# KudanLimited/cuda-bundle-adjustment

Hardware: AMD Instinct MI355X
Metric: ba_edge_iterations_per_sec (higher is better)
Workload: dtype f64

## Files before the change

cuda-bundle-adjustment_amd/csrc/host/engine.cpp:

```cpp
#include "engine.h"

#include <algorithm>
#include <atomic>
#include <chrono>
#include <cmath>
#include <cstring>
#include <cstdio>
#include <cstdlib>
#include <memory>
#include <thread>

#include "../kernels/kernels.h"
#include "chol_solver.h"
#include "edge_layout.h"
#include "hip_util.h"
#include "options.h"
#include "rccl_comm.h"
#include "relpose_plan.h"
#include "schur_plan.h"
#include "structure_gpu.h"
#include "thread_pool.h"

namespace cugo_host
{
// ... 1301 lines not shown
        m.pe.bind_relpose_plan(m.hsc_rowptr, m.hsc_colind, s, false);
    }
    m.begin_call(true);
    const Impl::CallFacts& f = m.f;
    Impl::LmState& st = m.st = Impl::LmState{};
    auto sync_prof = [&](int item, Clock::time_point t0) {
        if (m.profile)
        {
            CUGO_HIP(hipStreamSynchronize(s));
            prof_[item] += ms_since(t0);
        }
    };
    m.hash_begin(niterations);

    for (int iteration = 0; iteration < niterations; iteration++)
    {
        const auto it0 = Clock::now();
        auto tb = Clock::now();
        if (!st.spec_queued)
            m.queue_build(m.cur, f.can_fuse && iteration > 0 ? lambda : -1.0, iteration == 0 ? m.d_scal.data() : nullptr);
        st.spec_queued = false;
        sync_prof(PROF_BUILD_SYSTEM, tb);
        if (iteration == 0)
        {
            const double* hpp = m.d_Hpp.data();
            if (f.sharded)
            {
                CUGO_HIP(hipMemcpyAsync(m.d_tmp.data(), m.d_Hpp.data(), 36 * (size_t)m.P * sizeof(double),
                                        hipMemcpyDeviceToDevice, s));
                m.exchange(m.d_tmp.data(), 36 * (size_t)m.P, 0);
                hpp = m.d_tmp.data();
            }
            cugo_k::launch_max_diagonal(s, hpp, m.P, m.d_Hll.data(), m.L, m.rs(), m.d_scal.data() + 1);
            if (f.sharded)
            {
                m.exchange(m.d_scal.data(), 1, 0);
                m.exchange(m.d_scal.data() + 1, 1, 1);
            }
            CUGO_HIP(hipMemcpyAsync(m.h_scal.data(), m.d_scal.data(), 2 * sizeof(double), hipMemcpyDeviceToHost, s));
            CUGO_HIP(hipStreamSynchronize(s));
            F = m.h_scal[0];
            lambda = tau * m.h_scal[1];
        }

        int q = 0;
        double rho = -1.0;
        for (; q < maxq && rho < 0; q++)
        {
            const int hash_it = q == 0 ? iteration : -1;
            const bool trial_fused = q == 0 && st.fused_lambda == lambda;
            const bool one_stream = trial_fused && f.ps_on;
            if (st.spec_queued || (!one_stream && !st.hpp_valid))
            {
                m.queue_build(m.cur, -1.0);
                st.spec_queued = false;
            }
            m.hash(hash_it, 0, m.d_Hpp.data(), 36 * (size_t)m.P);
            m.hash(hash_it, 1, m.d_b.data(), 6 * (size_t)m.P + 3 * (size_t)m.L);
            m.hash(hash_it, 2, m.d_Hll.data(), 9 * (size_t)m.L);
            m.hash(hash_it, 3, m.d_Hpl.data(), f.blkw);
            auto ts = Clock::now();
            if (!(trial_fused && st.schur_lambda == lambda))
                m.queue_schur(lambda, trial_fused, one_stream, m.cur);
            st.schur_lambda = -1.0;
            if (f.sharded)
                m.exchange_system();
            sync_prof(PROF_SCHUR, ts);
            m.hash(hash_it, 4, m.d_sys.data(), 36 * (size_t)m.hs.n_blocks + 6 * (size_t)m.P);
            if (m.d_T.size())
                m.hash(hash_it, 5, m.d_T.data(), f.blkw);
            m.hash(hash_it, 6, m.d_invHll.data(), 9 * (size_t)m.L);
            auto tn = Clock::now();
            m.queue_factor_solve(lambda, hash_it);
            sync_prof(PROF_NUMERIC, tn);
            m.hash(hash_it, 7, m.xp(), 6 * (size_t)m.P);
            auto tu = Clock::now();
            const int nxt = m.cur ^ 1;
            int n_scale_part = 0;
            m.timed("backsubst_update", [&] {
                n_scale_part = cugo_k::launch_backsubst_update(
                    s, m.ev, lambda, (m.rank == 0 ? lambda : 0.0), m.d_invHll.data(), m.bl(), m.bp(),
                    one_stream ? m.d_T.data() : m.d_Hpl.data(), m.xp(), m.xl(), m.d_poses[m.cur].data(), m.d_lms[m.cur].data(),
                    m.d_poses[nxt].data(), m.d_lms[nxt].data(), m.rs(), f.sharded ? m.d_scal.data() + 3 : nullptr,
                    one_stream ? m.d_lmrec.data() : nullptr);
            });
            sync_prof(PROF_UPDATE, tu);
            m.hash(hash_it, 8, m.xl(), 3 * (size_t)m.L);
            m.hash(hash_it, 9, m.d_poses[nxt].data(), 7 * (size_t)m.Pall);
            m.hash(hash_it, 10, m.d_lms[nxt].data(), 3 * (size_t)m.Lall);
            auto te = Clock::now();
            const double lambda_pred = lambda * (1.0 / 3.0);
            const double fuse_pred = f.can_fuse ? lambda_pred : -1.0;
            const bool last = iteration + 1 == niterations;
            const bool from_build = f.from_build && q == 0 && !last && st.prev_clamped;
            if (from_build)
            {
                m.queue_build(nxt, fuse_pred, nullptr, true);
                m.timed("errors", [&] {
                    int n_icp_chi = 0;
                    const double* icp_chi = m.pe.chi_totals(&n_icp_chi);
                    cugo_k::launch_trial_tail_from_build(s, m.ev, m.rs(), n_scale_part, m.d_scal.data() + 2,
                                                         m.d_scal.data() + 4, m.h_scal.data() + 2, (double)++m.trial_seq,
                                                         reinterpret_cast<unsigned*>(m.d_fail.data() + 2), icp_chi,
                                                         n_icp_chi);
                });
                if (f.can_fuse)
                {
                    m.queue_schur(lambda_pred, true, f.ps_on, nxt);
                    st.schur_lambda = lambda_pred;
                }
                st.spec_queued = true;
            }
            else
            m.timed("errors", [&] {
                if (f.sharded)
                    cugo_k::launch_errors(s, m.ev, m.d_poses[nxt].data(), m.d_lms[nxt].data(), m.rk,
                                          m.rs(), m.d_scal.data() + 2);
                else
                {
                    int n_icp_chi = 0;
                    const double* icp_chi = m.pe.chi_totals(&n_icp_chi);
                    m.pe.queue_errors(s, m.d_poses[nxt].data());
                    cugo_k::launch_errors_tail(s, m.ev, m.d_poses[nxt].data(), m.d_lms[nxt].data(), m.rk, m.rs(),
                                               n_scale_part, m.d_scal.data() + 2, m.d_scal.data() + 4,
                                               m.h_scal.data() + 2, (double)++m.trial_seq,
                                               reinterpret_cast<unsigned*>(m.d_fail.data() + 2), icp_chi, n_icp_chi);
                }
            });
            m.last_err_buf = nxt;
            sync_prof(PROF_COMPUTE_ERROR, te);
            if (!from_build && f.speculate && q == 0 && !last)
            {
                if (!f.trial_poll && f.trial_event)
                {
                    if (!m.trial_ev)
                        CUGO_HIP(hipEventCreateWithFlags(&m.trial_ev, hipEventDisableTiming));
                    CUGO_HIP(hipEventRecord(m.trial_ev, s));
                }
                m.queue_build(nxt, fuse_pred);
                st.spec_queued = true;
            }
            const bool flag_summed = f.sharded && m.chol.own_subtrees();
            if (f.sharded)
            {
                if (flag_summed)
                    cugo_k::launch_flag_to_double(s, m.d_fail_flag());
                m.exchange(m.d_scal.data() + 2, flag_summed ? 3 : 2, 0);
                CUGO_HIP(hipMemcpyAsync(m.h_scal.data() + 2, m.d_scal.data() + 2, 3 * sizeof(double),
                                        hipMemcpyDeviceToHost, s));
            }
            m.wait_for_trial(st.spec_queued, sstats_.trial_sync_retries);
            int32_t fail_flag;
            std::memcpy(&fail_flag, m.h_scal.data() + 4, sizeof fail_flag);
            if (flag_summed)
                fail_flag = m.h_scal[4] > 0.5 ? 1 : 0;
            const bool success = fail_flag == 0;
            const double Fhat = m.h_scal[2];
            const double scale = (success ? m.h_scal[3] : 0.0) + 1e-3;
            const double Fdiff = Fhat - F;
            rho = success ? (F - Fhat) / scale : -1.0;
            if (!success)
                std::printf("factorize failed!\n");
            if (rho > 0)
            {
                const double a = 1 - std::pow(2 * rho - 1, 3);
                lambda *= std::max(1.0 / 3.0, std::min(a, 2.0 / 3.0));
                st.prev_clamped = a <= 1.0 / 3.0;
// ... 201 lines not shown
```

cuda-bundle-adjustment_amd/csrc/host/options.h:

```cpp
#pragma once
#include <cstdlib>

namespace cugo_host
{

struct Options
{
    int hsc_mfma = 1;
    bool hsc_xcd = true;
    bool hsc_rows = false, hsc_strip = false, schur_plan = false;
    bool fuse_t = true;
    bool pose_schur = true;
    bool float32 = false;
    bool speculate = true, trial_event = true, trial_poll = true;
    bool trial_from_build = true;
    bool profile = false;
    bool init_timing = false;
    bool structure_reuse = true;
    bool flatten_reuse = true;
    bool async_structure = true;
    bool host_structure = false;
    bool upload_thread = true;
    int own_subtrees = -1;
    double own_min_gflop = 3.0;
    bool lookahead = false;
    bool ea_lds = true, panel16 = true, asm_fronts = true;
    bool ea_direct = true;
    bool bw_chain = true;
    bool reduce_scatter = true;

    static Options from_env()
    {
        Options o;
        auto flag = [](const char* name) { return std::getenv(name) != nullptr; };
        auto off = [](const char* name) {
            const char* e = std::getenv(name);
            return e && e[0] == '0';
        };
        auto on = [](const char* name) {
            const char* e = std::getenv(name);
            return e && e[0] == '1';
        };
        if (const char* e = std::getenv("CUGO_HSC_MFMA"))
            o.hsc_mfma = e[0] == '0' ? 0 : e[0] == '2' ? 2 : 1;
        o.hsc_xcd = !off("CUGO_HSC_XCD");
        o.schur_plan = flag("CUGO_SCHUR_PLAN");
        o.hsc_rows = on("CUGO_HSC_ROWS"), o.hsc_strip = on("CUGO_HSC_STRIP");
        o.fuse_t = !off("CUGO_FUSE_T");
        o.pose_schur = !off("CUGO_POSE_SCHUR");
        o.float32 = on("CUGO_FLOAT32");
        o.speculate = !off("CUGO_SPECULATE"), o.trial_event = !off("CUGO_TRIAL_EVENT"), o.trial_poll = !off("CUGO_TRIAL_POLL");
        o.trial_from_build = !off("CUGO_TRIAL_FROM_BUILD");
        o.profile = flag("CUGO_PROFILE");
        o.init_timing = flag("CUGO_INIT_TIMING");
        o.structure_reuse = !flag("CUGO_NO_STRUCTURE_REUSE");
        o.flatten_reuse = !flag("CUGO_NO_FLATTEN_REUSE");
        o.async_structure = !off("CUGO_ASYNC_STRUCTURE");
        o.host_structure = flag("CUGO_HOST_STRUCTURE");
        o.upload_thread = !off("CUGO_UPLOAD_THREAD");
        if (const char* e = std::getenv("CUGO_OWN_SUBTREES"))
            o.own_subtrees = e[0] == '1' ? 1 : e[0] == '0' ? 0 : -1;
        if (const char* e = std::getenv("CUGO_OWN_MIN_GFLOP"))
            o.own_min_gflop = std::atof(e);
        if (const char* e = std::getenv("CUGO_LOOKAHEAD"))
            o.lookahead = std::atoi(e) != 0;
        o.ea_lds = !off("CUGO_EA_LDS"), o.panel16 = !off("CUGO_PANEL16"), o.asm_fronts = !off("CUGO_ASM_FRONTS");
        o.ea_direct = !off("CUGO_EA_DIRECT");
        o.bw_chain = !off("CUGO_BW_CHAIN");
        o.reduce_scatter = !off("CUGO_REDUCE_SCATTER");
        return o;
    }
};

}
```

cuda-bundle-adjustment_amd/csrc/kernels/ba_kernels.hip:

```cpp
#include "ba_math.h"
#include "kernels.h"

using namespace cugo_dev;

namespace
{

constexpr int BS = 256;

struct EV
{
    int E, Pall, Lall, P, L;
    const int32_t* pose;
    const int32_t* lm;
    const double* meas;
    const double* omega;
    int n_omega;
    const uint8_t* flags;
    const uint16_t* cam;
    const double* cams;
    int n_cams;
    const int32_t* lm_ptr;
    const int32_t* pose_ptr;
    const int32_t* pose_edge;
// ... 157 lines not shown
            if (blockIdx.x == 0)
                host_out[2] = *flag;
            __threadfence_system();
            if (atomicAdd(done, 1u) == 1u)
            {
                *done = 0u;
                __hip_atomic_store(host_out + 3, seq, __ATOMIC_RELEASE, __HIP_MEMORY_SCOPE_SYSTEM);
            }
        }
    }
}

__global__ __launch_bounds__(BS) void k_max_partials(const double* __restrict__ part, int n,
                                                     double* __restrict__ out)
{
    __shared__ double sm[BS];
    double v = 0;
    for (int i = threadIdx.x; i < n; i += BS)
        v = fmax(v, part[i]);
    sm[threadIdx.x] = v;
    __syncthreads();
    for (int s = BS / 2; s > 0; s >>= 1)
    {
        if ((int)threadIdx.x < s)
            sm[threadIdx.x] = fmax(sm[threadIdx.x], sm[threadIdx.x + s]);
        __syncthreads();
    }
    if (threadIdx.x == 0)
        out[0] = sm[0];
}

__global__ __launch_bounds__(BS) void k_errors(EV ev, const double* __restrict__ poses,
                                               const double* __restrict__ lms, Robust2 rk,
                                               double* __restrict__ partials)
{
    __shared__ double sm[BS / 64];
    const int e = blockIdx.x * BS + threadIdx.x;
    double chi = 0;
    if (e < ev.E)
    {
        const uint8_t fl = ev.flags[e];
        if (!(fl & CUGO_EDGE_INACTIVE))
        {
            const EdgeIn in = load_edge(ev, e, fl);
            EdgeGeom g;
            edge_residual(poses + 7 * (size_t)in.ip, lms + 3 * (size_t)in.il, in.mu, in.mv, in.mr,
                          in.stereo, in.omega, in.cam, in.stereo ? rk.s : rk.m, g);
            chi = g.chi;
        }
    }
    chi = block_sum(chi, sm);
    if (threadIdx.x == 0)
        partials[blockIdx.x] = chi;
}

__global__ __launch_bounds__(BS) void k_edge_chi(EV ev, const double* __restrict__ poses,
                                                 const double* __restrict__ lms, Robust2 rk,
                                                 double* __restrict__ chi_out)
{
    const int e = blockIdx.x * BS + threadIdx.x;
    if (e >= ev.E)
        return;
    const uint8_t fl = ev.flags[e];
    double chi = 0;
    if (!(fl & CUGO_EDGE_INACTIVE))
    {
        const EdgeIn in = load_edge(ev, e, fl);
        EdgeGeom g;
        edge_residual(poses + 7 * (size_t)in.ip, lms + 3 * (size_t)in.il, in.mu, in.mv, in.mr,
                      in.stereo, in.omega, in.cam, in.stereo ? rk.s : rk.m, g);
        chi = g.chi;
    }
    chi_out[e] = chi;
}

struct LmContrib
{
    double h00, h01, h02, h11, h12, h22, b0, b1, b2;
};
__device__ __forceinline__ LmContrib lm_contrib(const double JL[3][3], const EdgeGeom& g, bool stereo)
{
    const int dim = stereo ? 3 : 2;
    double s00 = 0, s01 = 0, s02 = 0, s11 = 0, s12 = 0, s22 = 0, t0 = 0, t1 = 0, t2 = 0;
    for (int m = 0; m < dim; m++)
    {
        s00 += JL[m][0] * JL[m][0];
        s01 += JL[m][0] * JL[m][1];
        s02 += JL[m][0] * JL[m][2];
        s11 += JL[m][1] * JL[m][1];
        s12 += JL[m][1] * JL[m][2];
        s22 += JL[m][2] * JL[m][2];
        t0 += JL[m][0] * g.e[m];
        t1 += JL[m][1] * g.e[m];
        t2 += JL[m][2] * g.e[m];
    }
    return LmContrib{g.w * s00, g.w * s01, g.w * s02, g.w * s11, g.w * s12, g.w * s22,
                     g.w * t0, g.w * t1, g.w * t2};
}

template <typename S>
__global__ __launch_bounds__(BS) void k_build_edges(EV ev, const double* __restrict__ poses,
                                                    const double* __restrict__ lms, Robust2 rk,
                                                    S* __restrict__ Hpl,
                                                    double* __restrict__ Hll,
                                                    double* __restrict__ bl,
                                                    double* __restrict__ rec,
                                                    double* __restrict__ partials,
                                                    double fuse_lambda, double* __restrict__ invHll,
                                                    S* __restrict__ T, double* __restrict__ lmrec)
{
    const bool fuse = fuse_lambda >= 0.0;
    const bool gform = fuse && T != nullptr && lmrec != nullptr;
    __shared__ double sm[BS / 64];
    __shared__ double2 pool2[BS * 9 + 1];
    double(*cs)[BS] = reinterpret_cast<double(*)[BS]>(pool2);
    double* rs_ = reinterpret_cast<double*>(pool2) + 9 * BS;
    double(*ivs)[7] = reinterpret_cast<double(*)[7]>(rs_);
    const int e = blockIdx.x * BS + threadIdx.x;
    double chi = 0;
    double H[18];
#pragma unroll
    for (int i = 0; i < 18; i++)
        H[i] = 0;
    LmContrib lc = {0, 0, 0, 0, 0, 0, 0, 0, 0};
    int l = -1;
    double r8[8] = {0, 0, 1, 0, 0, 0, 0, 0};
    if (e < ev.E)
    {
        const uint8_t fl = ev.flags[e];
        l = ev.lm[e];
        if (!(fl & CUGO_EDGE_INACTIVE))
        {
            const EdgeIn in = load_edge(ev, e, fl);
            const double* pose = poses + 7 * (size_t)in.ip;
            EdgeGeom g;
            edge_residual(pose, lms + 3 * (size_t)in.il, in.mu, in.mv, in.mr, in.stereo, in.omega,
                          in.cam, in.stereo ? rk.s : rk.m, g);
            chi = g.chi;
            r8[0] = g.Xc[0], r8[1] = g.Xc[1], r8[2] = g.Xc[2];
            r8[3] = g.e[0], r8[4] = g.e[1], r8[5] = g.e[2], r8[6] = g.w;
            const bool schur_act = !(fl & (CUGO_EDGE_FIXED_L | CUGO_EDGE_FIXED_P)) && l < ev.L;
            r8[7] = __longlong_as_double((long long)(ev.n_cams > 1 ? (int)ev.cam[e] : 0) |
                                         ((long long)(in.stereo ? 1 : 0) << 16) | ((long long)(schur_act ? 1 : 0) << 17) |
                                         ((long long)(schur_act ? l : 0) << 32));
            double JL[3][3];
            jac_landmark(g.Xc, pose, in.cam, in.stereo, JL);
            lc = lm_contrib(JL, g, in.stereo);
            if (!(fl & (CUGO_EDGE_FIXED_L | CUGO_EDGE_FIXED_P)))
            {
                double JP[3][6];
                jac_pose(g.Xc, in.cam, in.stereo, JP);
#pragma unroll
                for (int c = 0; c < 3; c++)
#pragma unroll
                    for (int r = 0; r < 6; r++)
                    {
                        double s = JP[0][r] * JL[0][c] + JP[1][r] * JL[1][c];
                        s += JP[2][r] * JL[2][c];
                        H[c * 6 + r] = g.w * s;
                    }
            }
        }
    }
    {
        const int t = threadIdx.x;
        cs[0][t] = lc.h00, cs[1][t] = lc.h01, cs[2][t] = lc.h02, cs[3][t] = lc.h11, cs[4][t] = lc.h12;
        cs[5][t] = lc.h22, cs[6][t] = lc.b0, cs[7][t] = lc.b1, cs[8][t] = lc.b2;
#pragma unroll
// ... 1595 lines not shown
                    }
                    const int uu = i / HR_PM, t = i - HR_PM * uu;
                    const int j = sdst[i];
                    const double* T = sT + uu * 18;
                    const double* H = sH + (uu * HR_SH + 1 + t) * 18;
                    double sp = T[r6] * H[c6];
                    sp = fma(T[6 + r6], H[6 + c6], sp);
                    sp = fma(T[12 + r6], H[12 + c6], sp);
                    if (lane < 36)
                        acc[36 * j + lane] += sp;
                }
            }
            if (!__syncthreads_or(np > t0 + HR_PM))
                break;
        }
    }
    if (lane < 36)
        dpart[w * 42 + lane] = dacc;
    else if (lane < 42)
        dpart[w * 42 + lane] = bacc;
    __syncthreads();
    if (tid < 36)
    {
        double sum = 0;
        for (int q = 0; q < HR_W; q++)
            sum += dpart[q * 42 + tid];
        double val = Hpp[36 * (size_t)p + tid] - sum;
        if (tid % 7 == 0)
            val += lambda_diag;
        Hsc[36 * (size_t)row0 + tid] = val;
    }
    else if (tid < 42)
    {
        double sum = 0;
        for (int q = 0; q < HR_W; q++)
            sum += dpart[q * 42 + tid];
        bsc[6 * (size_t)p + (tid - 36)] = bp[6 * (size_t)p + (tid - 36)] - sum;
    }
    for (int i = 36 + tid; i < 36 * nnz; i += HR_BS)
        Hsc[36 * (size_t)row0 + i] = -acc[i];
}

template <typename S>
__device__ __forceinline__ void hplT_x(const S* __restrict__ H, const double* __restrict__ x,
                                       double& s0, double& s1, double& s2)
{
    s0 = 0, s1 = 0, s2 = 0;
#pragma unroll
    for (int m = 0; m < 6; m++)
    {
        const double xm = x[m];
        s0 += (double)H[m] * xm;
        s1 += (double)H[6 + m] * xm;
        s2 += (double)H[12 + m] * xm;
    }
}

__device__ __forceinline__ void dev_update_poses(int blk, int nP, double lambda,
                                                 const double* __restrict__ xp,
                                                 const double* __restrict__ bp,
                                                 const double* __restrict__ poses_in,
                                                 double* __restrict__ poses_out,
                                                 double* __restrict__ partials, double* sm)
{
    const int p = blk * BS + threadIdx.x;
    double sc = 0;
    if (p < nP)
    {
        double dx[6];
#pragma unroll
        for (int i = 0; i < 6; i++)
        {
            dx[i] = xp[6 * (size_t)p + i];
            sc += dx[i] * (lambda * dx[i] + bp[6 * (size_t)p + i]);
        }
        pose_exp_update(dx, poses_in + 7 * (size_t)p, poses_out + 7 * (size_t)p);
    }
    sc = block_sum(sc, sm);
    if (threadIdx.x == 0)
        partials[blk] = sc;
}

template <typename S>
__global__ __launch_bounds__(BS) void k_backsubst_landmarks(
    EV ev, double lambda, const double* __restrict__ invHll, const double* __restrict__ bl,
    const S* __restrict__ Hpl, const double* __restrict__ xp, double* __restrict__ xl,
    const double* __restrict__ lms_in, double* __restrict__ lms_out,
    double* __restrict__ partials, int nbl, double lambda_pose, const double* __restrict__ bp,
    const double* __restrict__ poses_in, double* __restrict__ poses_out, const double* __restrict__ lmrec)
{
    __shared__ double sm[BS / 64];
    __shared__ double2 hs[BS * 9 + 1];
    double(*cs)[BS] = reinterpret_cast<double(*)[BS]>(hs);
    if ((int)blockIdx.x >= nbl)
    {
        dev_update_poses(blockIdx.x - nbl, ev.P, lambda_pose, xp, bp, poses_in, poses_out,
                         partials + nbl, sm);
        return;
    }
    const int t = threadIdx.x;
    const int ebase = blockIdx.x * BS;
    const int e = ebase + t;
    {
        const long nvalid = 9L * max(0, min(BS, ev.E - ebase));
        const size_t pbase = nvalid > 0 ? 9 * (size_t)ebase : 0;
        double2 v[9];
#pragma unroll
        for (int i = 0; i < 9; i++)
        {
            const int idx = i * BS + t;
            v[i] = ld_pair(Hpl, pbase + (size_t)min((long)idx, max(nvalid - 1, 0L)));
        }
#pragma unroll
        for (int i = 0; i < 9; i++)
            hs[i * BS + t] = v[i];
    }
    int l = -1;
    bool act = false;
    double x[6] = {0, 0, 0, 0, 0, 0};
    if (e < ev.E)
    {
        l = ev.lm[e];
        const uint8_t fl = ev.flags[e];
        act = !(fl & (CUGO_EDGE_FIXED_L | CUGO_EDGE_FIXED_P | CUGO_EDGE_INACTIVE));
        if (act)
        {
            const double2* px = reinterpret_cast<const double2*>(xp + 6 * (size_t)ev.pose[e]);
            const double2 a = px[0], b = px[1], c = px[2];
            x[0] = a.x, x[1] = a.y, x[2] = b.x, x[3] = b.y, x[4] = c.x, x[5] = c.y;
        }
    }
    __syncthreads();
    {
        double s0 = 0, s1 = 0, s2 = 0;
        if (act)
            hplT_x(reinterpret_cast<const double*>(hs) + 18 * t, x, s0, s1, s2);
        __syncthreads();
        cs[0][t] = s0, cs[1][t] = s1, cs[2][t] = s2;
    }
    __syncthreads();
    double sc = 0;
    if (l >= 0 && l < ev.L && ev.lm_ptr[l] == e)
    {
        const double b0 = bl[3 * (size_t)l], b1 = bl[3 * (size_t)l + 1], b2 = bl[3 * (size_t)l + 2];
        const double* lr = lmrec ? lmrec + 16 * (size_t)l : nullptr;
        double c0 = lr ? lr[6] : b0, c1 = lr ? lr[7] : b1, c2 = lr ? lr[8] : b2;
        const int e1 = ev.lm_ptr[l + 1];
        const int bend = min(e1, ebase + BS);
        for (int ee = e; ee < bend; ee++)
            c0 -= cs[0][ee - ebase], c1 -= cs[1][ee - ebase], c2 -= cs[2][ee - ebase];
        for (int ee = bend; ee < e1; ee++)
        {
            const uint8_t fl = ev.flags[ee];
            if (fl & (CUGO_EDGE_FIXED_L | CUGO_EDGE_FIXED_P | CUGO_EDGE_INACTIVE))
                continue;
            double s0, s1, s2;
            hplT_x(Hpl + 18 * (size_t)ee, xp + 6 * (size_t)ev.pose[ee], s0, s1, s2);
            c0 -= s0, c1 -= s1, c2 -= s2;
        }
        double x0, x1, x2;
        if (lr)
        {
            x0 = lr[0] * c0 + lr[1] * c1 + lr[3] * c2;
            x1 = lr[2] * c1 + lr[4] * c2;
            x2 = lr[5] * c2;
        }
        else
        {
            const double* iv = invHll + 9 * (size_t)l;
            x0 = iv[0] * c0 + iv[3] * c1 + iv[6] * c2;
            x1 = iv[1] * c0 + iv[4] * c1 + iv[7] * c2;
            x2 = iv[2] * c0 + iv[5] * c1 + iv[8] * c2;
        }
        xl[3 * (size_t)l] = x0, xl[3 * (size_t)l + 1] = x1, xl[3 * (size_t)l + 2] = x2;
        lms_out[3 * (size_t)l] = lms_in[3 * (size_t)l] + x0;
        lms_out[3 * (size_t)l + 1] = lms_in[3 * (size_t)l + 1] + x1;
        lms_out[3 * (size_t)l + 2] = lms_in[3 * (size_t)l + 2] + x2;
        sc = x0 * (lambda * x0 + b0) + x1 * (lambda * x1 + b1) + x2 * (lambda * x2 + b2);
    }
    if (e < ev.L && ev.lm_ptr[e] == ev.lm_ptr[e + 1])
    {
        xl[3 * (size_t)e] = 0, xl[3 * (size_t)e + 1] = 0, xl[3 * (size_t)e + 2] = 0;
        lms_out[3 * (size_t)e] = lms_in[3 * (size_t)e];
        lms_out[3 * (size_t)e + 1] = lms_in[3 * (size_t)e + 1];
        lms_out[3 * (size_t)e + 2] = lms_in[3 * (size_t)e + 2];
    }
    sc = block_sum(sc, sm);
    if (threadIdx.x == 0)
        partials[blockIdx.x] = sc;
}

inline int div_up(long a, int b) { return (int)((a + b - 1) / b); }

}

namespace cugo_k
{

static LaunchHook* g_hook = nullptr;
void set_launch_hook(LaunchHook* h) { g_hook = h; }
LaunchHook* launch_hook() { return g_hook; }

static size_t spec_chi_offset(int n_edges, int n_poses, int n_landmarks)
{
    return (size_t)div_up(n_edges > n_landmarks ? n_edges : n_landmarks, BS) + div_up(n_poses, BS) + 64;
}
static size_t scratch_partials(int n_edges, int n_poses, int n_landmarks)
{
    const size_t n = 2 * (size_t)div_up(n_edges > n_landmarks ? n_edges : n_landmarks, BS) + div_up(n_poses, BS) + 4096;
    return (n + 31) & ~size_t(31);
}
size_t reduce_scratch_doubles(int n_edges, int n_poses, int n_landmarks)
{
    return scratch_partials(n_edges, n_poses, n_landmarks) + 8 * ((size_t)n_edges + BS);
}
// ... 147 lines not shown
    if (hs.n_blocks > 0 && rows.d_off_pi && hs.d_rowptr && ev.P > 0)
    {
        static bool attr_set[2] = {false, false};
        if (!attr_set[sizeof(S) == 4])
        {
            (void)hipFuncSetAttribute(reinterpret_cast<const void*>(k_hsc_offdiag_strip<S>),
                                      hipFuncAttributeMaxDynamicSharedMemorySize, (int)hs_lds_bytes());
            attr_set[sizeof(S) == 4] = true;
        }
        CUGO_LAUNCH_T(k_hsc_offdiag_strip, S, dim3(xcd_grid(ev.P)), dim3(HS_BS), hs_lds_bytes(), s, ev, hs.d_rowptr,
                      hs.d_off_ptr, hs.d_off_ei, rows.d_off_pi, hs.d_off_ej, d_Hpl, (const S*)d_T, d_Hsc);
    }
    else if (hs.n_blocks > 0 && rows.mfma)
    {
        ::cugo_k::LaunchScope _scope("k_hsc_offdiag_mfma", s);
        if (rows.xcd)
            hipLaunchKernelGGL((k_hsc_offdiag_mfma<S, true>), dim3(xcd_grid(div_up(hs.n_blocks, BS / 64))), dim3(BS), 0, s,
                               hs.n_blocks, hs.d_off_ptr, hs.d_off_ei, hs.d_off_ej, d_Hpl_off, (const S*)d_T, d_Hsc);
        else
            hipLaunchKernelGGL((k_hsc_offdiag_mfma<S, false>), dim3(div_up(hs.n_blocks, BS / 64)), dim3(BS), 0, s,
                               hs.n_blocks, hs.d_off_ptr, hs.d_off_ei, hs.d_off_ej, d_Hpl_off, (const S*)d_T, d_Hsc);
    }
    else if (hs.n_blocks > 0)
        CUGO_LAUNCH_T(k_hsc_offdiag, S, dim3(div_up(hs.n_blocks, BS / 64)), dim3(BS), 0, s,
                      hs.n_blocks, hs.d_off_ptr, hs.d_off_ei, hs.d_off_ej, d_Hpl_off, (const S*)d_T, d_Hsc);
    if (ev.P > 0 && have_T && rows.d_lmrec)
    {
        const double* d_rec = rows.rs.d_partials + scratch_partials(ev.E, ev.P, ev.L);
        CUGO_LAUNCH(k_pose_schur, dim3(xcd_grid(ev.P)), dim3(PS_BS), 0, s, ev, d_rec, rows.d_lmrec, rows.d_poses,
                      hs.d_rowptr, damp_hsc_diag ? lambda : 0.0, d_Hsc, rows.d_bp_out, d_bsc);
    }
    else if (ev.P > 0 && rows.mfma == 1)
        CUGO_LAUNCH_T(k_hsc_diag_mfma, S, dim3(xcd_grid(ev.P)), dim3(HM_BS), 0, s, ev,
                      hs.d_rowptr, damp_hsc_diag ? lambda : 0.0, d_Hpp, d_bp, d_bl, d_Hpl, (const S*)d_T,
                      d_Hsc, d_bsc);
    else if (ev.P > 0)
        CUGO_LAUNCH_T(k_hsc_diag, S, dim3(xcd_grid(ev.P)), dim3(HD_BS), 0, s, ev,
                      hs.d_rowptr, damp_hsc_diag ? lambda : 0.0, d_Hpp, d_bp, d_bl, d_Hpl, (const S*)d_T,
                      d_Hsc, d_bsc);
}

void launch_schur(hipStream_t s, const cugo_edges& e, const cugo_hsc_struct& hs, double lambda,
                  int damp_hsc_diag, const double* d_Hpp, const double* d_bp, const double* d_Hll,
                  const double* d_bl, const void* d_Hpl, double* d_invHll, void* d_T,
                  double* d_bsc, double* d_Hsc, bool have_T, SchurRows rows)
{
    if (e.block_f32)
        launch_schur_t(s, e, hs, lambda, damp_hsc_diag, d_Hpp, d_bp, d_Hll, d_bl,
                       static_cast<const float*>(d_Hpl), d_invHll, static_cast<float*>(d_T), d_bsc, d_Hsc, have_T, rows);
    else
        launch_schur_t(s, e, hs, lambda, damp_hsc_diag, d_Hpp, d_bp, d_Hll, d_bl,
                       static_cast<const double*>(d_Hpl), d_invHll, static_cast<double*>(d_T), d_bsc, d_Hsc, have_T, rows);
}

bool schur_rows_usable(const cugo_hsc_struct& hs, int max_row_nnz)
{
    const size_t lds = (36 * (size_t)std::max(max_row_nnz, 1) + hr_fixed_doubles()) * sizeof(double);
    return hs.d_rowptr && hs.d_colind && lds <= 150 * 1024;
}

void launch_list_pos(hipStream_t s, const cugo_edges& e, int n_list, size_t M, const int32_t* d_off_ei,
                     int32_t* d_pose_pos, int32_t* d_off_pi)
{
    const EV ev = make_ev(e);
    if (n_list > 0)
        CUGO_LAUNCH(k_pose_pos, dim3(div_up(n_list, BS)), dim3(BS), 0, s, ev, n_list, d_pose_pos);
    if (M > 0)
        CUGO_LAUNCH(k_list_pos, dim3((unsigned)((M + BS - 1) / BS)), dim3(BS), 0, s, M, d_off_ei, (const int32_t*)d_pose_pos,
                    d_off_pi);
}

void launch_pose_rec(hipStream_t s, const cugo_edges& e, int n, int32_t* d_rec)
{
    const EV ev = make_ev(e);
    if (n > 0)
        CUGO_LAUNCH(k_pose_rec, dim3(div_up(n, BS)), dim3(BS), 0, s, ev, n, reinterpret_cast<int4*>(d_rec));
}

template <typename S>
static int launch_backsubst_update_t(hipStream_t s, const cugo_edges& e, double lambda, double lambda_pose,
                                      const double* d_invHll, const double* d_bl, const double* d_bp,
                                      const S* d_Hpl, const double* d_xp, double* d_xl,
                                      const double* d_poses_in, const double* d_lms_in, double* d_poses_out,
                                      double* d_lms_out, ReduceScratch rs, double* d_scale, const double* d_lmrec)
{
    const EV ev = make_ev(e);
    const int nbl = div_up(ev.E > ev.L ? ev.E : ev.L, BS), nbp = div_up(ev.P, BS);
    if (nbl + nbp > 0)
        CUGO_LAUNCH_T(k_backsubst_landmarks, S, dim3(nbl + nbp), dim3(BS), 0, s, ev, lambda, d_invHll,
                      d_bl, d_Hpl, d_xp, d_xl, d_lms_in, d_lms_out, rs.d_partials, nbl,
                      lambda_pose, d_bp, d_poses_in, d_poses_out, d_lmrec);
    if (d_scale)
        CUGO_LAUNCH(k_sum_partials, dim3(1), dim3(SP_BS), 0, s, rs.d_partials, nbl + nbp, d_scale);
    return nbl + nbp;
}

int launch_backsubst_update(hipStream_t s, const cugo_edges& e, double lambda, double lambda_pose,
                            const double* d_invHll, const double* d_bl, const double* d_bp,
                            const void* d_Hpl, const double* d_xp, double* d_xl,
                            const double* d_poses_in, const double* d_lms_in, double* d_poses_out,
                            double* d_lms_out, ReduceScratch rs, double* d_scale, const double* d_lmrec)
{
    if (e.block_f32)
        return launch_backsubst_update_t(s, e, lambda, lambda_pose, d_invHll, d_bl, d_bp, static_cast<const float*>(d_Hpl),
                                  d_xp, d_xl, d_poses_in, d_lms_in, d_poses_out, d_lms_out, rs, d_scale, d_lmrec);
    return launch_backsubst_update_t(s, e, lambda, lambda_pose, d_invHll, d_bl, d_bp, static_cast<const double*>(d_Hpl),
                                  d_xp, d_xl, d_poses_in, d_lms_in, d_poses_out, d_lms_out, rs, d_scale, d_lmrec);
}

}
```

cuda-bundle-adjustment_amd/csrc/kernels/ba_math.h:

```cpp
#pragma once
#include <hip/hip_runtime.h>
#include <stdint.h>

namespace cugo_dev
{

struct Robust
{
    int type;
    double delta;
};

__device__ __forceinline__ double rk_rho(const Robust rk, double x)
{
    const double d2 = rk.delta * rk.delta;
    if (rk.type == 2)
    {
        const double u = 1.0 - x / d2;
        const double mx = (1.0 / 3) * d2;
        return x <= d2 ? mx * (1.0 - u * u * u) : mx;
    }
    if (rk.type == 1)
        return d2 * log((1.0 / d2) * x + 1.0);
    if (rk.type == 3)
// ... 115 lines not shown
        const double iZZ = invZ * invZ, bf = cam[4];
        JP[0][0] = X * Y * iZZ * fu;
        JP[0][1] = -(1 + (X * X * iZZ)) * fu;
        JP[0][2] = Y * invZ * fu;
        JP[0][3] = -1 * invZ * fu;
        JP[0][4] = 0;
        JP[0][5] = X * iZZ * fu;
        JP[1][0] = (1 + Y * Y * iZZ) * fv;
        JP[1][1] = -X * Y * iZZ * fv;
        JP[1][2] = -X * invZ * fv;
        JP[1][3] = 0;
        JP[1][4] = -1 * invZ * fv;
        JP[1][5] = Y * iZZ * fv;
        JP[2][0] = JP[0][0] - bf * Y * iZZ;
        JP[2][1] = JP[0][1] + bf * X * iZZ;
        JP[2][2] = JP[0][2];
        JP[2][3] = JP[0][3];
        JP[2][4] = 0;
        JP[2][5] = JP[0][5] - bf * iZZ;
    }
}

__device__ __forceinline__ void jac_landmark_R(const double* Xc, const double R[3][3],
                                               const double* __restrict__ cam, bool stereo,
                                               double JL[3][3])
{
    const double X = Xc[0], Y = Xc[1], Z = Xc[2];
    const double invZ = 1.0 / Z;
    const double fu = cam[0], fv = cam[1];
    if (!stereo)
    {
        const double x = invZ * X, y = invZ * Y;
        const double fu_iz = fu * invZ, fv_iz = fv * invZ;
#pragma unroll
        for (int j = 0; j < 3; j++)
        {
            JL[0][j] = -fu_iz * (R[0][j] - x * R[2][j]);
            JL[1][j] = -fv_iz * (R[1][j] - y * R[2][j]);
            JL[2][j] = 0;
        }
    }
    else
    {
        const double iZZ = invZ * invZ, bf = cam[4];
#pragma unroll
        for (int j = 0; j < 3; j++)
        {
            JL[0][j] = -fu * R[0][j] * invZ + fu * X * R[2][j] * iZZ;
            JL[1][j] = -fv * R[1][j] * invZ + fv * Y * R[2][j] * iZZ;
            JL[2][j] = JL[0][j] - bf * R[2][j] * iZZ;
        }
    }
}
__device__ __forceinline__ void jac_landmark(const double* Xc, const double* __restrict__ q,
                                             const double* __restrict__ cam, bool stereo,
                                             double JL[3][3])
{
    double R[3][3];
    quat_to_rot(q, R);
    jac_landmark_R(Xc, R, cam, stereo, JL);
}

struct Sym3
{
    double b00, b01, b02, b11, b12, b22;
};
__device__ __forceinline__ Sym3 sym3_inv(const double* __restrict__ A, double lambda)
{
    const double A00 = A[0] + lambda, A01 = A[3], A11 = A[4] + lambda;
    const double A02 = A[2], A12 = A[7], A22 = A[8] + lambda;
    const double det = A00 * A11 * A22 + A01 * A12 * A02 + A02 * A01 * A12 - A00 * A12 * A12 -
                       A02 * A11 * A02 - A01 * A01 * A22;
    const double id = 1 / det;
    Sym3 s;
    s.b00 = id * (A11 * A22 - A12 * A12);
    s.b01 = id * (A02 * A12 - A01 * A22);
    s.b11 = id * (A00 * A22 - A02 * A02);
    s.b02 = id * (A01 * A12 - A02 * A11);
    s.b12 = id * (A02 * A01 - A00 * A12);
    s.b22 = id * (A00 * A11 - A01 * A01);
    return s;
}

__device__ __forceinline__ void pose_exp_update(const double* __restrict__ dx,
                                                const double* __restrict__ pin,
                                                double* __restrict__ pout)
{
    const double wx = dx[0], wy = dx[1], wz = dx[2];
    const double theta = sqrt(wx * wx + wy * wy + wz * wz);
    double a1, a2, b1, b2;
    if (theta < 0.00001)
    {
        a1 = 1.0, a2 = 0.5, b1 = 0.5, b2 = 1.0 / 6;
    }
    else
    {
        a1 = sin(theta) / theta;
        a2 = (1 - cos(theta)) / (theta * theta);
        b1 = a2;
        b2 = (theta - sin(theta)) / (theta * theta * theta);
    }
    const double xx = wx * wx, yy = wy * wy, zz = wz * wz;
    const double xy = wx * wy, yz = wy * wz, zx = wz * wx;
    const double O1[3][3] = {{0, -wz, wy}, {wz, 0, -wx}, {-wy, wx, 0}};
    const double O2[3][3] = {{-yy - zz, xy, zx}, {xy, -zz - xx, yz}, {zx, yz, -xx - yy}};
    double R[3][3], V[3][3];
#pragma unroll
    for (int i = 0; i < 3; i++)
#pragma unroll
        for (int j = 0; j < 3; j++)
        {
            const double I = (i == j) ? 1.0 : 0.0;
            R[i][j] = I + a1 * O1[i][j] + a2 * O2[i][j];
            V[i][j] = I + b1 * O1[i][j] + b2 * O2[i][j];
        }
    double dq[4];
    double t = R[0][0] + R[1][1] + R[2][2];
    if (t > 0)
    {
        t = sqrt(t + 1);
        dq[3] = 0.5 * t;
        t = 0.5 / t;
        dq[0] = (R[2][1] - R[1][2]) * t;
        dq[1] = (R[0][2] - R[2][0]) * t;
        dq[2] = (R[1][0] - R[0][1]) * t;
    }
    else
    {
        int i = 0;
        if (R[1][1] > R[0][0])
            i = 1;
        if (R[2][2] > R[i][i])
            i = 2;
        const int j = (i + 1) % 3, k = (j + 1) % 3;
        t = sqrt(R[i][i] - R[j][j] - R[k][k] + 1);
        dq[i] = 0.5 * t;
        t = 0.5 / t;
        dq[3] = (R[k][j] - R[j][k]) * t;
        dq[j] = (R[j][i] + R[i][j]) * t;
        dq[k] = (R[k][i] + R[i][k]) * t;
    }
    const double dt0 = V[0][0] * dx[3] + V[0][1] * dx[4] + V[0][2] * dx[5];
    const double dt1 = V[1][0] * dx[3] + V[1][1] * dx[4] + V[1][2] * dx[5];
    const double dt2 = V[2][0] * dx[3] + V[2][1] * dx[4] + V[2][2] * dx[5];
    const double q0 = pin[0], q1 = pin[1], q2 = pin[2], q3 = pin[3];
    const double tx = pin[4], ty = pin[5], tz = pin[6];
    double c1x = dq[1] * tz - dq[2] * ty;
    double c1y = dq[2] * tx - dq[0] * tz;
    double c1z = dq[0] * ty - dq[1] * tx;
    c1x += c1x;
    c1y += c1y;
    c1z += c1z;
    const double c2x = dq[1] * c1z - dq[2] * c1y;
    const double c2y = dq[2] * c1x - dq[0] * c1z;
    const double c2z = dq[0] * c1y - dq[1] * c1x;
    pout[4] = dt0 + (tx + dq[3] * c1x + c2x);
    pout[5] = dt1 + (ty + dq[3] * c1y + c2y);
    pout[6] = dt2 + (tz + dq[3] * c1z + c2z);
    double r3 = dq[3] * q3 - dq[0] * q0 - dq[1] * q1 - dq[2] * q2;
    double r0 = dq[3] * q0 + dq[0] * q3 + dq[1] * q2 - dq[2] * q1;
    double r1 = dq[3] * q1 + dq[1] * q3 + dq[2] * q0 - dq[0] * q2;
    double r2 = dq[3] * q2 + dq[2] * q3 + dq[0] * q1 - dq[1] * q0;
    double invn = 1 / sqrt(r0 * r0 + r1 * r1 + r2 * r2 + r3 * r3);
    if (r3 < 0)
        invn = -invn;
    pout[0] = invn * r0;
    pout[1] = invn * r1;
    pout[2] = invn * r2;
    pout[3] = invn * r3;
}

__device__ __forceinline__ void tri6_unpack(int t, int& r, int& c)
{
    r = 0;
    int k = t;
    while (k >= 6 - r)
        k -= 6 - r, r++;
    c = r + k;
}
template <bool SCHUR>
__device__ __forceinline__ void pose_term_add(int p, int t, int r, int c, double s, double* __restrict__ H,
                                              const int32_t* __restrict__ rowptr, double* __restrict__ bp,
                                              double* __restrict__ bsc)
{
    if (t < 21)
    {
        double* blk = H + 36 * (size_t)(SCHUR ? rowptr[p] : p);
        blk[r + 6 * c] += s;
        if (r != c)
            blk[c + 6 * r] += s;
    }
    else if (t < 27)
    {
        bp[6 * (size_t)p + (t - 21)] += s;
        if (SCHUR)
            bsc[6 * (size_t)p + (t - 21)] += s;
    }
}

}
```

cuda-bundle-adjustment_amd/csrc/kernels/kernels.h:

```cpp
#pragma once
#include <hip/hip_runtime.h>
#include <stddef.h>
#include <stdint.h>

#include "../../../include/cugo_hip.h"

namespace cugo_k
{

struct LaunchHook
{
    virtual void begin(const char* kernel, hipStream_t s) = 0;
    virtual void end(const char* kernel, hipStream_t s) = 0;
    virtual ~LaunchHook() {}
};
void set_launch_hook(LaunchHook* h);
LaunchHook* launch_hook();
struct LaunchScope
{
    const char* name;
    hipStream_t s;
    LaunchHook* h;
    LaunchScope(const char* n, hipStream_t st) : name(n), s(st), h(launch_hook())
    {
        if (h)
            h->begin(name, s);
    }
    ~LaunchScope()
    {
        if (h)
            h->end(name, s);
    }
};
#define CUGO_LAUNCH(kernel, grid, block, lds, stream, ...)                          \
    do                                                                              \
    {                                                                               \
        ::cugo_k::LaunchScope _scope(#kernel, stream);                              \
        hipLaunchKernelGGL(kernel, grid, block, lds, stream, __VA_ARGS__);          \
    } while (0)

struct ReduceScratch
{
    double* d_partials;
    size_t capacity;
};

void launch_errors(hipStream_t s, const cugo_edges& ev, const double* d_poses, const double* d_lms,
                   cugo_robust rk, ReduceScratch rs, double* d_chi);

void launch_build(hipStream_t s, const cugo_edges& ev, const double* d_poses, const double* d_lms,
                  cugo_robust rk, double* d_Hpp, double* d_bp, double* d_Hll, double* d_bl,
                  void* d_Hpl, ReduceScratch rs, double* d_chi, double fuse_lambda = -1.0,
                  double* d_invHll = nullptr, void* d_T = nullptr, double* d_lmrec = nullptr, bool skip_poses = false,
                  bool chi_behind_scale = false);

void launch_trial_tail_from_build(hipStream_t s, const cugo_edges& ev, ReduceScratch rs, int n_scale_partials,
                                  double* d_out, const double* d_flag, double* h_out, double seq, unsigned* d_done,
                                  const double* d_icp_chi = nullptr, int n_icp_chi = 0);

void launch_max_diagonal(hipStream_t s, const double* d_Hpp, int nP, const double* d_Hll, int nL,
                         ReduceScratch rs, double* d_out);

struct SchurRows
{
    const int32_t* d_pose_rec = nullptr;
    int max_row_nnz = 0;
    const int32_t* d_off_pi = nullptr;
    int mfma = 1;
    bool xcd = true;
    const double* d_lmrec = nullptr;
    const double* d_poses = nullptr;
    ReduceScratch rs{nullptr, 0};
    double* d_bp_out = nullptr;
};
void launch_list_pos(hipStream_t s, const cugo_edges& ev, int n_list, size_t M, const int32_t* d_off_ei,
                     int32_t* d_pose_pos, int32_t* d_off_pi);
void launch_pose_rec(hipStream_t s, const cugo_edges& ev, int n, int32_t* d_rec);
bool schur_rows_usable(const cugo_hsc_struct& hs, int max_row_nnz);
void launch_schur(hipStream_t s, const cugo_edges& ev, const cugo_hsc_struct& hs, double lambda,
                  int damp_hsc_diag, const double* d_Hpp, const double* d_bp, const double* d_Hll,
                  const double* d_bl, const void* d_Hpl, double* d_invHll, void* d_T,
                  double* d_bsc, double* d_Hsc, bool have_T = false, SchurRows rows = SchurRows());

int launch_backsubst_update(hipStream_t s, const cugo_edges& ev, double lambda, double lambda_pose,
                            const double* d_invHll, const double* d_bl, const double* d_bp,
                            const void* d_Hpl, const double* d_xp, double* d_xl,
                            const double* d_poses_in, const double* d_lms_in, double* d_poses_out,
                            double* d_lms_out, ReduceScratch rs, double* d_scale,
                            const double* d_lmrec = nullptr);
void launch_errors_tail(hipStream_t s, const cugo_edges& ev, const double* d_poses, const double* d_lms,
                        cugo_robust rk, ReduceScratch rs, int n_scale_partials, double* d_out,
                        const double* d_flag, double* h_out, double seq, unsigned* d_done,
                        const double* d_icp_chi = nullptr, int n_icp_chi = 0);

size_t reduce_scratch_doubles(int n_edges, int n_poses, int n_landmarks);

void launch_pose_chi_total(hipStream_t s, const char* label, const double* d_totals, int n, double* d_chi, bool chi_add);
struct PoseIndexCheck
{
    const int32_t *d_pose, *d_pose_ptr;
    int n;
    const char* label;
};
int pose_check_indices(hipStream_t s, const char* who, const PoseIndexCheck* kinds, int n_kinds, int n_poses_total, int* d_bad);

size_t icp_scratch_doubles(const cugo_icp_edges& ev);
void launch_icp_build(hipStream_t s, const cugo_icp_edges& ev, const double* d_poses, double* d_Hpp, double* d_bp,
                      ReduceScratch rs, double* d_chi, bool chi_add = false);
void launch_icp_errors(hipStream_t s, const cugo_icp_edges& ev, const double* d_poses, ReduceScratch rs, double* d_chi,
                       bool chi_add = false, double* d_edge_chi = nullptr);
void launch_icp_chunks(hipStream_t s, const cugo_icp_edges& ev, const double* d_poses, bool full, ReduceScratch rs,
                       double* d_edge_chi = nullptr);
void launch_icp_add(hipStream_t s, const cugo_icp_edges& ev, ReduceScratch rs, double* d_Hpp, double* d_bp);
void launch_icp_add_schur(hipStream_t s, const cugo_icp_edges& ev, ReduceScratch rs, const int32_t* d_rowptr,
                          double* d_Hsc, double* d_bp, double* d_bsc);
int icp_chunk_count(const cugo_icp_edges& ev);

int prior_workgroups(const cugo_prior_edges& ev);
void launch_prior_errors(hipStream_t s, const cugo_prior_edges& ev, const double* d_poses, double* d_wg_chi,
                         double* d_edge_chi = nullptr);
void launch_prior_add(hipStream_t s, const cugo_prior_edges& ev, const double* d_poses, double* d_Hpp, double* d_bp,
                      double* d_wg_chi);
void launch_prior_add_schur(hipStream_t s, const cugo_prior_edges& ev, const double* d_poses, const int32_t* d_rowptr,
                            double* d_Hsc, double* d_bp, double* d_bsc, double* d_wg_chi);

struct RelPosePlanDev
{
    int n, n_poses_free;
    const int32_t *pose_a, *pose_b;
    const int32_t *inc_ptr, *inc;
    const int32_t* off_blk;
};
int relpose_workgroups(const cugo_relpose_edges& ev);
void launch_relpose_errors(hipStream_t s, const cugo_relpose_edges& ev, const RelPosePlanDev& plan, const double* d_poses,
                           double* d_wg_chi, double* d_edge_chi = nullptr);
void launch_relpose_add(hipStream_t s, const cugo_relpose_edges& ev, const RelPosePlanDev& plan, const double* d_poses,
                        double* d_Hpp, double* d_bp, double* d_Hoff, double* d_wg_chi);
void launch_relpose_add_schur(hipStream_t s, const cugo_relpose_edges& ev, const RelPosePlanDev& plan, const double* d_poses,
                              const int32_t* d_rowptr, double* d_Hsc, double* d_bp, double* d_bsc, double* d_wg_chi);
void launch_relpose_add_offdiag(hipStream_t s, const cugo_relpose_edges& ev, const RelPosePlanDev& plan, const double* d_poses,
                                double* d_Hsc);

void launch_edge_chi(hipStream_t s, const cugo_edges& e, const double* d_poses, const double* d_lms,
                     cugo_robust rk, double* d_chi_e);

constexpr int TMETA = 36;
constexpr int EA1_REC = 16;
struct CholPlanDev
{
    int n_fronts;
    const int32_t* ncb;
    const int32_t* nb;
    const int64_t* off;
    const int64_t* ldf;
    const int32_t* alias_of;
    const int32_t* bw_np;
    const int32_t* la_np;
    const int64_t* woff;
    double* winv;
    const int64_t* l21off;
    double* l21;
    int nc_max;
    int ea_lds;
    int panel16;
    int ea_direct;
#ifdef CUGO_DEBUG_HOOKS
    int kernel_acquire;
    int dbg_delay;
    int zero_lds;
    int lds_doubles;
    int dbg_skip_wg;
#endif
// ... 87 lines not shown
```

Baseline: 641.3 million.

## Recompute Hpl products in back-substitution from compact per-edge records

Adds a record-based path to the landmark back-substitution kernel. It loads 8-double per-edge records (camera-frame point, weight, camera/stereo bits) from scratch space and recomputes the Jacobians to form the Hpl^T x product, instead of reading the stored 9-wide Hpl blocks. This cuts global-memory traffic in exchange for extra FP64 arithmetic. The change also fully unrolls the landmark contribution loop and replaces the dynamic-index quaternion-from-rotation branch with templated specializations so array indexing is static.

```diff
diff --git a/cuda-bundle-adjustment_amd/csrc/host/engine.cpp b/cuda-bundle-adjustment_amd/csrc/host/engine.cpp
--- a/cuda-bundle-adjustment_amd/csrc/host/engine.cpp
+++ b/cuda-bundle-adjustment_amd/csrc/host/engine.cpp
@@ -1407,7 +1407,7 @@
                     s, m.ev, lambda, (m.rank == 0 ? lambda : 0.0), m.d_invHll.data(), m.bl(), m.bp(),
                     one_stream ? m.d_T.data() : m.d_Hpl.data(), m.xp(), m.xl(), m.d_poses[m.cur].data(), m.d_lms[m.cur].data(),
                     m.d_poses[nxt].data(), m.d_lms[nxt].data(), m.rs(), f.sharded ? m.d_scal.data() + 3 : nullptr,
-                    one_stream ? m.d_lmrec.data() : nullptr);
+                    one_stream ? m.d_lmrec.data() : nullptr, one_stream && m.opt.bs_records);
             });
             sync_prof(PROF_UPDATE, tu);
             m.hash(hash_it, 8, m.xl(), 3 * (size_t)m.L);
diff --git a/cuda-bundle-adjustment_amd/csrc/host/options.h b/cuda-bundle-adjustment_amd/csrc/host/options.h
--- a/cuda-bundle-adjustment_amd/csrc/host/options.h
+++ b/cuda-bundle-adjustment_amd/csrc/host/options.h
@@ -12,6 +12,7 @@
     bool fuse_t = true;
     bool pose_schur = true;
     bool float32 = false;
+    bool bs_records = true;
     bool speculate = true, trial_event = true, trial_poll = true;
     bool trial_from_build = true;
     bool profile = false;
@@ -49,6 +50,7 @@
         o.fuse_t = !off("CUGO_FUSE_T");
         o.pose_schur = !off("CUGO_POSE_SCHUR");
         o.float32 = on("CUGO_FLOAT32");
+        o.bs_records = !off("CUGO_BS_RECORDS");
         o.speculate = !off("CUGO_SPECULATE"), o.trial_event = !off("CUGO_TRIAL_EVENT"), o.trial_poll = !off("CUGO_TRIAL_POLL");
         o.trial_from_build = !off("CUGO_TRIAL_FROM_BUILD");
         o.profile = flag("CUGO_PROFILE");
diff --git a/cuda-bundle-adjustment_amd/csrc/kernels/ba_kernels.hip b/cuda-bundle-adjustment_amd/csrc/kernels/ba_kernels.hip
--- a/cuda-bundle-adjustment_amd/csrc/kernels/ba_kernels.hip
+++ b/cuda-bundle-adjustment_amd/csrc/kernels/ba_kernels.hip
@@ -263,8 +263,11 @@
 {
     const int dim = stereo ? 3 : 2;
     double s00 = 0, s01 = 0, s02 = 0, s11 = 0, s12 = 0, s22 = 0, t0 = 0, t1 = 0, t2 = 0;
-    for (int m = 0; m < dim; m++)
-    {
+#pragma unroll
+    for (int m = 0; m < 3; m++)
+    {
+        if (m >= dim)
+            continue;
         s00 += JL[m][0] * JL[m][0];
         s01 += JL[m][0] * JL[m][1];
         s02 += JL[m][0] * JL[m][2];
@@ -2026,16 +2029,53 @@
 }
 
 template <typename S>
+__device__ __forceinline__ void gT_x_from_record(const double* r8, const double* __restrict__ pose,
+                                                 const double* __restrict__ cams, const double* __restrict__ q,
+                                                 const double* x, double& s0, double& s1, double& s2)
+{
+    const double Xc[3] = {r8[0], r8[1], r8[2]};
+    const double w = r8[6];
+    const long long bits = __double_as_longlong(r8[7]);
+    const double* cam = cams + 5 * (int)(bits & 0xffff);
+    const bool stereo = ((bits >> 16) & 1) != 0;
+    double JL[3][3], JP[3][6];
+    jac_landmark(Xc, pose, cam, stereo, JL);
+    jac_pose(Xc, cam, stereo, JP);
+    const double q0 = q[0], q1 = q[1], q2 = q[2], q3 = q[3], q4 = q[4], q5 = q[5];
+    s0 = 0, s1 = 0, s2 = 0;
+#pragma unroll
+    for (int m = 0; m < 6; m++)
+    {
+        double h[3];
+#pragma unroll
+        for (int c = 0; c < 3; c++)
+        {
+            double s = JP[0][m] * JL[0][c] + JP[1][m] * JL[1][c];
+            s += JP[2][m] * JL[2][c];
+            h[c] = w * s;
+        }
+        const double g0 = (double)(S)(h[0] * q0);
+        const double g1 = (double)(S)(h[0] * q1 + h[1] * q2);
+        const double g2 = (double)(S)(h[0] * q3 + h[1] * q4 + h[2] * q5);
+        const double xm = x[m];
+        s0 += g0 * xm;
+        s1 += g1 * xm;
+        s2 += g2 * xm;
+    }
+}
+
+template <typename S, bool REC>
 __global__ __launch_bounds__(BS) void k_backsubst_landmarks(
     EV ev, double lambda, const double* __restrict__ invHll, const double* __restrict__ bl,
     const S* __restrict__ Hpl, const double* __restrict__ xp, double* __restrict__ xl,
     const double* __restrict__ lms_in, double* __restrict__ lms_out,
     double* __restrict__ partials, int nbl, double lambda_pose, const double* __restrict__ bp,
-    const double* __restrict__ poses_in, double* __restrict__ poses_out, const double* __restrict__ lmrec)
+    const double* __restrict__ poses_in, double* __restrict__ poses_out, const double* __restrict__ lmrec,
+    const double* __restrict__ rec)
 {
     __shared__ double sm[BS / 64];
-    __shared__ double2 hs[BS * 9 + 1];
-    double(*cs)[BS] = reinterpret_cast<double(*)[BS]>(hs);
+    __shared__ double2 hs[REC ? BS * 6 : BS * 9 + 1];
+    double(*cs)[BS] = reinterpret_cast<double(*)[BS]>(reinterpret_cast<double*>(hs) + (REC ? 9 * BS : 0));
     if ((int)blockIdx.x >= nbl)
     {
         dev_update_poses(blockIdx.x - nbl, ev.P, lambda_pose, xp, bp, poses_in, poses_out,
@@ -2045,6 +2085,25 @@
     const int t = threadIdx.x;
     const int ebase = blockIdx.x * BS;
     const int e = ebase + t;
+    if constexpr (REC)
+    {
+        double* rs_ = reinterpret_cast<double*>(hs);
+        const long base = 8L * ebase, limit = 8L * ev.E;
+        double2 v[4];
+#pragma unroll
+        for (int i = 0; i < 4; i++)
+        {
+            const int f = 2 * (i * BS + t);
+            v[i] = base + f < limit ? *reinterpret_cast<const double2*>(rec + base + f) : make_double2(0, 0);
+        }
+#pragma unroll
+        for (int i = 0; i < 4; i++)
+        {
+            const int f = 2 * (i * BS + t);
+            rs_[9 * (f >> 3) + (f & 7)] = v[i].x, rs_[9 * (f >> 3) + (f & 7) + 1] = v[i].y;
+        }
+    }
+    else
     {
         const long nvalid = 9L * max(0, min(BS, ev.E - ebase));
         const size_t pbase = nvalid > 0 ? 9 * (size_t)ebase : 0;
@@ -2075,6 +2134,15 @@
         }
     }
     __syncthreads();
+    if constexpr (REC)
+    {
+        double s0 = 0, s1 = 0, s2 = 0;
+        if (act && l < ev.L)
+            gT_x_from_record<S>(reinterpret_cast<const double*>(hs) + 9 * t, poses_in + 7 * (size_t)ev.pose[e], ev.cams,
+                                lmrec + 16 * (size_t)l, x, s0, s1, s2);
+        cs[0][t] = s0, cs[1][t] = s1, cs[2][t] = s2;
+    }
+    else
     {
         double s0 = 0, s1 = 0, s2 = 0;
         if (act)
@@ -2388,14 +2456,24 @@
                                       const double* d_invHll, const double* d_bl, const double* d_bp,
                                       const S* d_Hpl, const double* d_xp, double* d_xl,
                                       const double* d_poses_in, const double* d_lms_in, double* d_poses_out,
-                                      double* d_lms_out, ReduceScratch rs, double* d_scale, const double* d_lmrec)
+                                      double* d_lms_out, ReduceScratch rs, double* d_scale, const double* d_lmrec,
+                                      bool from_records)
 {
     const EV ev = make_ev(e);
     const int nbl = div_up(ev.E > ev.L ? ev.E : ev.L, BS), nbp = div_up(ev.P, BS);
     if (nbl + nbp > 0)
-        CUGO_LAUNCH_T(k_backsubst_landmarks, S, dim3(nbl + nbp), dim3(BS), 0, s, ev, lambda, d_invHll,
-                      d_bl, d_Hpl, d_xp, d_xl, d_lms_in, d_lms_out, rs.d_partials, nbl,
-                      lambda_pose, d_bp, d_poses_in, d_poses_out, d_lmrec);
+    {
+        ::cugo_k::LaunchScope _scope("k_backsubst_landmarks", s);
+        const double* d_rec = rs.d_partials + scratch_partials(ev.E, ev.P, ev.L);
+        if (from_records && d_lmrec)
+            hipLaunchKernelGGL((k_backsubst_landmarks<S, true>), dim3(nbl + nbp), dim3(BS), 0, s, ev, lambda, d_invHll,
+                               d_bl, d_Hpl, d_xp, d_xl, d_lms_in, d_lms_out, rs.d_partials, nbl, lambda_pose, d_bp,
+                               d_poses_in, d_poses_out, d_lmrec, d_rec);
+        else
+            hipLaunchKernelGGL((k_backsubst_landmarks<S, false>), dim3(nbl + nbp), dim3(BS), 0, s, ev, lambda, d_invHll,
+                               d_bl, d_Hpl, d_xp, d_xl, d_lms_in, d_lms_out, rs.d_partials, nbl, lambda_pose, d_bp,
+                               d_poses_in, d_poses_out, d_lmrec, d_rec);
+    }
     if (d_scale)
         CUGO_LAUNCH(k_sum_partials, dim3(1), dim3(SP_BS), 0, s, rs.d_partials, nbl + nbp, d_scale);
     return nbl + nbp;
@@ -2405,13 +2483,14 @@
                             const double* d_invHll, const double* d_bl, const double* d_bp,
                             const void* d_Hpl, const double* d_xp, double* d_xl,
                             const double* d_poses_in, const double* d_lms_in, double* d_poses_out,
-                            double* d_lms_out, ReduceScratch rs, double* d_scale, const double* d_lmrec)
+                            double* d_lms_out, ReduceScratch rs, double* d_scale, const double* d_lmrec,
+                            bool from_records)
 {
     if (e.block_f32)
         return launch_backsubst_update_t(s, e, lambda, lambda_pose, d_invHll, d_bl, d_bp, static_cast<const float*>(d_Hpl),
-                                  d_xp, d_xl, d_poses_in, d_lms_in, d_poses_out, d_lms_out, rs, d_scale, d_lmrec);
+                                  d_xp, d_xl, d_poses_in, d_lms_in, d_poses_out, d_lms_out, rs, d_scale, d_lmrec, from_records);
     return launch_backsubst_update_t(s, e, lambda, lambda_pose, d_invHll, d_bl, d_bp, static_cast<const double*>(d_Hpl),
-                                  d_xp, d_xl, d_poses_in, d_lms_in, d_poses_out, d_lms_out, rs, d_scale, d_lmrec);
-}
-
-}
+                                  d_xp, d_xl, d_poses_in, d_lms_in, d_poses_out, d_lms_out, rs, d_scale, d_lmrec, from_records);
+}
+
+}
diff --git a/cuda-bundle-adjustment_amd/csrc/kernels/ba_math.h b/cuda-bundle-adjustment_amd/csrc/kernels/ba_math.h
--- a/cuda-bundle-adjustment_amd/csrc/kernels/ba_math.h
+++ b/cuda-bundle-adjustment_amd/csrc/kernels/ba_math.h
@@ -221,6 +221,18 @@
     return s;
 }
 
+template <int I>
+__device__ __forceinline__ void quat_of_rot_diag(const double R[3][3], double dq[4])
+{
+    constexpr int J = (I + 1) % 3, K = (J + 1) % 3;
+    double t = sqrt(R[I][I] - R[J][J] - R[K][K] + 1);
+    dq[I] = 0.5 * t;
+    t = 0.5 / t;
+    dq[3] = (R[K][J] - R[J][K]) * t;
+    dq[J] = (R[J][I] + R[I][J]) * t;
+    dq[K] = (R[K][I] + R[I][K]) * t;
+}
+
 __device__ __forceinline__ void pose_exp_update(const double* __restrict__ dx,
                                                 const double* __restrict__ pin,
                                                 double* __restrict__ pout)
@@ -266,18 +278,14 @@
     }
     else
     {
-        int i = 0;
-        if (R[1][1] > R[0][0])
-            i = 1;
-        if (R[2][2] > R[i][i])
-            i = 2;
-        const int j = (i + 1) % 3, k = (j + 1) % 3;
-        t = sqrt(R[i][i] - R[j][j] - R[k][k] + 1);
-        dq[i] = 0.5 * t;
-        t = 0.5 / t;
-        dq[3] = (R[k][j] - R[j][k]) * t;
-        dq[j] = (R[j][i] + R[i][j]) * t;
-        dq[k] = (R[k][i] + R[i][k]) * t;
+        const bool c1 = R[1][1] > R[0][0];
+        const bool c2 = R[2][2] > (c1 ? R[1][1] : R[0][0]);
+        if (c2)
+            quat_of_rot_diag<2>(R, dq);
+        else if (c1)
+            quat_of_rot_diag<1>(R, dq);
+        else
+            quat_of_rot_diag<0>(R, dq);
     }
     const double dt0 = V[0][0] * dx[3] + V[0][1] * dx[4] + V[0][2] * dx[5];
     const double dt1 = V[1][0] * dx[3] + V[1][1] * dx[4] + V[1][2] * dx[5];
diff --git a/cuda-bundle-adjustment_amd/csrc/kernels/kernels.h b/cuda-bundle-adjustment_amd/csrc/kernels/kernels.h
--- a/cuda-bundle-adjustment_amd/csrc/kernels/kernels.h
+++ b/cuda-bundle-adjustment_amd/csrc/kernels/kernels.h
@@ -87,7 +87,8 @@
                             const void* d_Hpl, const double* d_xp, double* d_xl,
                             const double* d_poses_in, const double* d_lms_in, double* d_poses_out,
                             double* d_lms_out, ReduceScratch rs, double* d_scale,
-                            const double* d_lmrec = nullptr);
+                            const double* d_lmrec = nullptr,
+                            bool from_records = false);
 void launch_errors_tail(hipStream_t s, const cugo_edges& ev, const double* d_poses, const double* d_lms,
                         cugo_robust rk, ReduceScratch rs, int n_scale_partials, double* d_out,
                         const double* d_flag, double* h_out, double seq, unsigned* d_done,
```

Result: faster. 652.8 million (median of 6 runs) (+1.8%).
